# jamornsriwasansak/smallpt-enoki-optix

Hardware: AMD Instinct MI355X
Metric: Mpaths/sec (pixels x spp / s), mitsuba.obj-standin 1024^2 x 64spp, depth 8 (higher is better)
Workload: dtype f32

## Files before the change

include/spt.h:

```cpp
#ifndef SPT_H
#define SPT_H

#include <stddef.h>
#include <stdint.h>

#ifdef __cplusplus
extern "C" {
#endif

typedef int32_t spt_status;
enum {
    SPT_OK = 0,
    SPT_ERR_INVALID = 1,
    SPT_ERR_HIP = 2,
    SPT_ERR_NO_DEVICE = 3,
    SPT_ERR_OOM = 4,
    SPT_ERR_IO = 5,
    SPT_ERR_LIMIT = 6
};

typedef struct spt_scene_t* spt_scene;

typedef struct spt_rays {
    const float* ox; const float* oy; const float* oz;
// ... 22 lines not shown
    float fov_y;
    float film_size_y;
} spt_camera;

enum {
    SPT_RNG_Y_FIRST = 0,
    SPT_RNG_X_FIRST = 1
};

enum {
    SPT_FLAG_TIMING = 1u,
    SPT_FLAG_TRAVERSAL_STATS = 2u,
    SPT_FLAG_FUSED = 4u,
    SPT_FLAG_WAVEFRONT = 8u,
    SPT_FLAG_TIMING_ALL = 16u,
    SPT_FLAG_NO_BOUNCE_CULL = 32u
};

typedef struct spt_render_params {
    uint32_t width, height;
    uint32_t spp;
    uint32_t max_depth;
    spt_camera camera;
    uint32_t tile_index, tile_count, rows_per_group;
    uint32_t wavefront_paths;
    uint32_t rr_start_depth;
    uint32_t rng_order;
    uint64_t rng_initstate;
    float env[3];
    uint32_t flags;
} spt_render_params;
// ... 291 lines not shown

spt_status spt_scene_isect_busy_begin(spt_scene scene);
spt_status spt_scene_isect_busy_end(spt_scene scene, double* busy_ms, uint64_t* launches);
enum { SPT_KERNEL_ISECT = 1u, SPT_KERNEL_DRAIN = 2u };
spt_status spt_scene_kernel_busy(spt_scene scene, uint32_t kernels, double* busy_ms, uint64_t* launches);

uint32_t spt_tile_rows(uint32_t height, uint32_t tile_index, uint32_t tile_count,
                       uint32_t rows_per_group, uint32_t* rows, uint32_t cap);

void spt_default_params(spt_render_params* p);

const char* spt_last_error(void);
const char* spt_version(void);
const char* spt_build_id(void);
void spt_debug_fail_workspace_alloc(int32_t nth);

spt_status spt_obj_load(const char* path, spt_mesh* out);
void spt_mesh_free(spt_mesh* mesh);

typedef struct spt_pbrt_info {
    uint32_t has_camera;
    spt_camera camera;
    float fov_deg;
    uint32_t xres, yres;
    uint32_t has_env;
    float env[3];
    uint64_t shapes;
    uint64_t shapes_skipped;
    uint64_t instances;
} spt_pbrt_info;
// ... 14 lines not shown
```

smallpt-enoki-optix_amd/csrc/kernels.hip:

```cpp
#include <hipcub/hipcub.hpp>
#include <type_traits>

#include "spt_internal.h"

namespace spt {

__device__ __forceinline__ uint32_t wave_uniform(uint32_t v) { return __builtin_amdgcn_readfirstlane(v); }

typedef float spt_f4v __attribute__((ext_vector_type(4)));
typedef float spt_f2v __attribute__((ext_vector_type(2)));
template <bool kNt = false>
__device__ __forceinline__ float4 ldq(const float4* p) {
    if constexpr (kNt) {
        const spt_f4v v = __builtin_nontemporal_load((const spt_f4v*)p);
        return make_float4(v.x, v.y, v.z, v.w);
    } else {
        return *p;
    }
}
template <bool kNt = false>
__device__ __forceinline__ void stq(float4* p, float4 x) {
    if constexpr (kNt) {
        spt_f4v v = {x.x, x.y, x.z, x.w};
        __builtin_nontemporal_store(v, (spt_f4v*)p);
// ... 292 lines not shown
        o = o_;
        const float dx = fabsf(d.x) < kMinDir ? copysignf(kMinDir, d.x) : d.x;
        const float dy = fabsf(d.y) < kMinDir ? copysignf(kMinDir, d.y) : d.y;
        const float dz = fabsf(d.z) < kMinDir ? copysignf(kMinDir, d.z) : d.z;
        ix = __builtin_amdgcn_rcpf(dx); iy = __builtin_amdgcn_rcpf(dy); iz = __builtin_amdgcn_rcpf(dz);
        const uint32_t oct = (ix < 0.0f ? 1u : 0u) | (iy < 0.0f ? 2u : 0u) | (iz < 0.0f ? 4u : 0u);
        const uint32_t oct_inv = oct ^ 7u;
        const uint32_t kz = k >> 4;
        oct_rep = oct_inv * 0x01010101u | ((kz == 2u ? 0u : kz + 1u) << 3);
        tmin = tmin_;
        tbox = box_tmin(tmin_);
        nhits = 1u << (24u + oct_inv);
        ht = tmax_;
    }

    __device__ __forceinline__ bool root_misses(const DeviceScene& sc) {
        nhits = 0;
        tbase = 0;
        thits = 0;
        tbase2 = 0;
        thits2 = 0;
        const uint4* np = sc.nodes8;
        const uint4 w0 = np[0], w1 = np[1], w2 = np[2], w3 = np[3];
        if constexpr (kW == 6) visit_words6(w0, w1, w2, w3);
        else visit_words(w0, w1, w2, w3, np[4]);
        return !(thits | (nhits & 0xff000000u));
    }

    __device__ __forceinline__ void init(const DeviceScene& sc, V3 o_, V3 d, float tmin_, float tmax_, bool anyhit_,
                                         const Lds& L) {
        wr = woop_setup(o_, d);
        spa = (L.wbase + lane_id()) * 4u;
        *wrec(sc, L) = make_uint4(f2u(wr.Sx), f2u(wr.Sy), f2u(wr.Sz), wr.k);
        uint32_t none, zero;
        asm volatile("v_mov_b32 %0, -1" : "=v"(none));
        asm volatile("v_mov_b32 %0, 0" : "=v"(zero));
        *hrec(sc, L) = make_uint4(none, none, zero, zero);
        init_slabs(o_, d, tmin_, tmax_, wr.k);
        anyhit = anyhit_;
        tbase = 0;
        thits = 0;
        tbase2 = 0;
        thits2 = 0;
        done = sc.empty != 0;
    }

    __device__ __forceinline__ uint32_t octx(uint32_t mw) const {
        const uint32_t t8 = mw & (mw >> 1) & 0x08080808u;
        return mw ^ ((t8 - (t8 >> 3)) & oct_rep);
    }

    __device__ __forceinline__ void take_hits(uint32_t hm, uint32_t group, uint32_t tri_base) {
        nhits = (hm & 0xff000000u) | group;
        if (thits) {
            tbase2 = tri_base;
            thits2 = hm & 0x00ffffffu;
// ... 637 lines not shown
        if (!kSpt) {
            const Frame fr = frame_from_normal(sn);
            nd = to_world(fr, cosine_hemisphere(xi_x, xi_y));
        } else {
            float wgt;
            nd = scatter(a.sc, kind, slot, d, no, sn, xi_x, xi_y, wgt);
            tr = tr * wgt; tg = tg * wgt; tb = tb * wgt;
        }
    }
    if constexpr (kCull) {
        __shared__ uint32_t s_wave_cull[kBlock / 64];
        bool gone = false;
        if (emit) {
            CullTr ct;
            ct.init_slabs(no, nd, kRayTmin, kRayTmax, CullTr::kNoRot);
            gone = ct.root_misses(a.sc);
            emit = !gone;
        }
        const uint64_t gball = __ballot(gone);
        if (lane == 0) s_wave_cull[wave] = (uint32_t)__popcll(gball);
        rank = compact_block<kBlock>(a, emit, s_wave_cnt, tid, lane, wave, base);
        if (tid == 0) {
            uint32_t n = 0;
            for (uint32_t w = 0; w < kBlock / 64; w++) n += s_wave_cull[w];
            if (n) atomicAdd(culled + (blockIdx.x % kShards) * kCullStride, (unsigned long long)n);
        }
        if (gone)
            a.sflag[film_slot((meta >> kMetaDepthBits) - a.sample0, pix, a.P, a.chunk_ns, a.work_order)] = 1;
    }
    if (tid == 0) {
        uint32_t off = base;
        for (uint32_t w = 0; w < kBlock / 64; w++) {
            s_wave_off[w] = off;
            off += s_wave_cnt[w];
        }
    }
    __syncthreads();
    if (emit) store_path<kMode, kNt>(a.out, s_wave_off[wave] + rank, no, nd, pix, meta + 1u, tr, tg, tb, lr, lg, lb);
}

template <int kMode, bool kSpt, bool kNt = false>
__global__ __launch_bounds__(kShadeBlock) void shade_kernel(ShadeArgs a) {
    const uint32_t n = *a.count_in;
    if (n < a.drain_below) return;
    const uint32_t nreal = min(gridDim.x, (n + kShadeBlock - 1) / kShadeBlock);
    const uint32_t i =
        (a.xcd_remap && blockIdx.x < nreal ? xcd_block(blockIdx.x, nreal) : blockIdx.x) * kShadeBlock + threadIdx.x;
    shade_block<kMode, kSpt, kNt, kShadeBlock>(a, i < n, QueueSrc<kNt>{a, i});
}

struct CamSrc {
    V3 o, d;
    uint32_t pix, meta;
// ... 100 lines not shown
        dep = dep + t;
        cov = cov + c;
    }
    const float fs = (float)a.spp;
    if (a.albedo_r) a.albedo_r[p] = ar / fs;
    if (a.albedo_g) a.albedo_g[p] = ag / fs;
    if (a.albedo_b) a.albedo_b[p] = ab / fs;
    if (a.normal_x) a.normal_x[p] = nx / fs;
    if (a.normal_y) a.normal_y[p] = ny / fs;
    if (a.normal_z) a.normal_z[p] = nz / fs;
    if (a.depth) a.depth[p] = dep / fs;
    if (a.coverage) a.coverage[p] = cov / fs;
}

template <typename Tr, int kMode, bool kDrain = false, bool kNt = false, bool kList = false, bool kEnv = false,
          bool kNee = false, bool kSky = false, bool kMis = false>
__global__ __launch_bounds__(kIsectBlock)
__attribute__((amdgpu_waves_per_eu(kDrain && kMode == kModeUnit ? (kNt ? SPT_DRAIN_WAVES_NT : SPT_DRAIN_WAVES)
                                   : kDrain ? SPT_DRAIN_WAVES_RGB : SPT_FUSED_WAVES, 8)))
void render_fused_kernel(FusedArgs a) {
    constexpr bool kEmit = kMode == kModeEmit;
    static_assert(!kNee || (kEmit && !kDrain), "light sampling: emitter mode, not the drain");
    static_assert(!kSky || (kNee && kEnv), "sky sampling: the light-sampling lane loop of a scene with a sky image");
    static_assert(!kMis || kNee, "MIS: between the shadow rays and the bounce rays of the light-sampling lane loop");
#if SPT_WAVE_LOG
    const unsigned long long wl_t0 = (unsigned long long)wall_clock64();
#endif
    extern __shared__ uint32_t lds_stack[];
    const Lds L = block_lds(lds_stack);
    uint32_t n = a.count;
    if constexpr (kDrain) {
        if (a.seg_count) {
            n = 0;
            for (uint32_t j = 0; j < kShards; j++) n += a.seg_count[j * kShardStride];
            n = wave_uniform(n);
        } else {
// ... 215 lines not shown
                                        if (traced) {
                                            park[2] = make_float4(dir.x, dir.y, dir.z, sc3.x);
                                            park[3] = make_float4(sc3.y, sc3.z, u2f(lid), 0.0f);
                                            dir = sd;
                                            shadow = true;
                                        }
                                    }
                                }
                            }
                            meta++;
                            if constexpr (kPark) {
                                park[0] = make_float4(thr, thg, thb, lr);
                                park[1] = make_float4(lg, lb, kNee ? u2f(nee_prev) : 0.0f, kMis ? cb : 0.0f);
                            }
                            tr.o = hp;
                            need_init = true;
                            busy = true;
                            cont = true;
                        }
                    }
                }
                if (term) {
                    if (kMode == kModeUnit) {
                        a.sflag[film_slot(sample - a.sample0, pix, a.P, a.pm_ns, a.pm_ns != 0)] = slot == -1 ? 1 : 0;
                    } else {
                        size_t cs;
                        float* f = film_rgb(a.sfilm, sample - a.sample0, pix, a.P, a.pm_ns, a.pm_ns != 0, cs);
                        f[0] = lr;
                        f[cs] = lg;
                        f[2 * cs] = lb;
// ... 28 lines not shown
                        xcd_tries++;
                    }
                    if (xcd_tries >= 8u) { drained = true; break; }
                } else if (pool == pool_end) {
                    uint32_t base = 0;
                    if ((threadIdx.x & 63u) == 0) base = atomicAdd(a.next, a.chunk);
                    base = dyn_base + wave_uniform((uint32_t)__shfl((int)base, 0));
                    if (base >= n) { drained = true; break; }
                    pool = base;
                    pool_end = min(base + a.chunk, n);
                }
                const uint32_t rank = __builtin_amdgcn_mbcnt_hi((uint32_t)(idle >> 32),
                                                                __builtin_amdgcn_mbcnt_lo((uint32_t)idle, 0u));
                const uint32_t take = min((uint32_t)__popcll(idle), pool_end - pool);
                if (kDrain && !busy && !pending && rank < take) {
                    const uint32_t j = a.perm ? a.perm[pool + rank] : pool + rank;
                    const float4 q1 = ldq<kNt>(a.q.q1 + j), q2 = ldq<kNt>(a.q.q2 + j);
                    meta = f2u(q1.w);
                    pix = f2u(q2.w);
                    dir = v3(q2.x, q2.y, q2.z);
                    thr = thg = thb = 1.0f;
                    lr = lg = lb = 0.0f;
                    if (kMode >= kModeAlbedo) {
                        const float4 q0 = ldq<kNt>(a.q.q0 + j);
                        thr = q0.x; thg = q0.y; thb = q0.z;
                        if (kEmit) lr = q0.w;
                    }
                    if (kEmit) {
                        const float2 l = ldq2<kNt>(a.q.rad + j);
                        lg = l.x; lb = l.y;
                    }
                    if constexpr (kPark) {
// ... 27 lines not shown
                }
                if (!kDrain) starts += take;
                pool += take;
#if SPT_WAVE_LOG
                ph[6] += take;
#endif
                idle = __ballot(!busy && !pending);
            }
            if (need_init) {
                if constexpr (kNee) {
                    float tmn = kRayTmin, tmx = kRayTmax;
                    if (shadow) light_shadow_interval(dir, tmn, tmx);
                    if constexpr (kSky)
                        if (skyray) sky_shadow_interval(dir, tmn, tmx);
                    tr.init(a.sc, tr.o, dir, tmn, tmx, kSky && skyray, L);
                } else {
                    tr.init(a.sc, tr.o, dir, kRayTmin, kRayTmax,
                            (meta & ((1u << kMetaDepthBits) - 1u)) + 1u >= a.max_depth && !kEmit, L);
                }
                if (tr.finished()) {
                    busy = false;
                    pending = true;
                }
            }
#if SPT_WAVE_LOG
            const unsigned long long ph_t3 = __builtin_readcyclecounter();
            ph[1] += ph_t3 - ph_t0;
            ph[7] += ph_t3 - ph_t2;
#endif
        }
// ... 521 lines not shown
        else if (mode == kModeEmit) hipLaunchKernelGGL((shade_kernel<kModeEmit, false, true>), g, b, 0, s, a);
        else if (mode == kModeAlbedo && spt) hipLaunchKernelGGL((shade_kernel<kModeAlbedo, true, true>), g, b, 0, s, a);
        else if (mode == kModeAlbedo) hipLaunchKernelGGL((shade_kernel<kModeAlbedo, false, true>), g, b, 0, s, a);
        else hipLaunchKernelGGL((shade_kernel<kModeUnit, false, true>), g, b, 0, s, a);
        return hipGetLastError();
    }
    if (mode == kModeEmit && spt) hipLaunchKernelGGL((shade_kernel<kModeEmit, true>), g, b, 0, s, a);
    else if (mode == kModeEmit) hipLaunchKernelGGL((shade_kernel<kModeEmit, false>), g, b, 0, s, a);
    else if (mode == kModeAlbedo && spt) hipLaunchKernelGGL((shade_kernel<kModeAlbedo, true>), g, b, 0, s, a);
    else if (mode == kModeAlbedo) hipLaunchKernelGGL((shade_kernel<kModeAlbedo, false>), g, b, 0, s, a);
    else hipLaunchKernelGGL((shade_kernel<kModeUnit, false>), g, b, 0, s, a);
    return hipGetLastError();
}

template <typename Tr, int kMode, bool kDrain = false, bool kNt = false, bool kList = false, bool kEnv = false,
          bool kNee = false, bool kSky = false, bool kMis = false>
static hipError_t launch_fused_t(const FusedArgs& a, hipStream_t s, uint32_t* lanes_out) {
    static thread_local size_t cached_lds = 0;
    static thread_local uint32_t cached = 0;
    static thread_local int cached_dev = -1;
    const size_t park = kMode != kModeUnit ? (size_t)kIsectBlock * (kNee ? 64 : 32) : 0;
    const size_t lds = (size_t)a.sc.stack_depth * Tr::kStackWords * kIsectBlock * sizeof(uint32_t) + Tr::kExtraLds + park;
    int dev = 0;
    (void)hipGetDevice(&dev);
    if (!cached || cached_lds != lds || cached_dev != dev) {
        int per_cu = 0, cus = 0;
        if (hipOccupancyMaxActiveBlocksPerMultiprocessor(&per_cu, render_fused_kernel<Tr, kMode, kDrain, kNt, kList, kEnv, kNee, kSky, kMis>,
                                                         kIsectBlock, lds) != hipSuccess || per_cu <= 0)
            per_cu = 1;
        if (hipDeviceGetAttribute(&cus, hipDeviceAttributeMultiprocessorCount, dev) != hipSuccess || cus <= 0)
            cus = 256;
        cached = (uint32_t)(per_cu * cus);
        cached_lds = lds;
        cached_dev = dev;
    }
    const uint32_t scaled = a.grid_q8 ? max(1u, (uint32_t)(((uint64_t)cached * a.grid_q8) >> 8)) : cached;
    const uint32_t blocks = kDrain ? scaled : min(scaled, blocks_for(a.count > 0 ? a.count : 1, kIsectBlock));
    if (lanes_out) *lanes_out = blocks * kIsectBlock;
    hipLaunchKernelGGL((render_fused_kernel<Tr, kMode, kDrain, kNt, kList, kEnv, kNee, kSky, kMis>), dim3(blocks), dim3(kIsectBlock),
                       lds, s, a);
    return hipGetLastError();
}

template <typename Tr, int kMode, bool kDrain = false, bool kNt = false, bool kList = false>
static hipError_t launch_fused_e(const FusedArgs& a, hipStream_t s, uint32_t* lanes_out) {
    if constexpr (kMode == kModeEmit && !kDrain && !kNt) {
        if (a.sc.sky && a.sc.envmap) {
            if (a.sc.mis) return launch_fused_t<Tr, kMode, kDrain, kNt, kList, true, true, true, true>(a, s, lanes_out);
            return launch_fused_t<Tr, kMode, kDrain, kNt, kList, true, true, true>(a, s, lanes_out);
        }
        if (a.sc.lights) {
            if (a.sc.envmap) {
                if (a.sc.mis) return launch_fused_t<Tr, kMode, kDrain, kNt, kList, true, true, false, true>(a, s, lanes_out);
                return launch_fused_t<Tr, kMode, kDrain, kNt, kList, true, true>(a, s, lanes_out);
// ... 60 lines not shown
    if (e) return e;
    return hipcub::DeviceRadixSort::SortPairs(tmp, *tmp_bytes, keys, keys_out, vals, perm, (int)cap, 0, 30, s);
}

hipError_t launch_drain(const FusedArgs& a, int mode, hipStream_t s) {
    if (a.nt) {
        if (mode == kModeEmit) return launch_drain_m<kModeEmit, true>(a, s);
        if (mode == kModeAlbedo) return launch_drain_m<kModeAlbedo, true>(a, s);
        return launch_drain_m<kModeUnit, true>(a, s);
    }
    if (mode == kModeEmit) return launch_drain_m<kModeEmit, false>(a, s);
    if (mode == kModeAlbedo) return launch_drain_m<kModeAlbedo, false>(a, s);
    return launch_drain_m<kModeUnit, false>(a, s);
}

template <typename Tr>
static hipError_t launch_fused_list(const FusedArgs& a, int mode, hipStream_t s, uint32_t* lanes_out) {
    if (mode == kModeEmit) return launch_fused_e<Tr, kModeEmit, false, false, true>(a, s, lanes_out);
    if (mode == kModeAlbedo) return launch_fused_e<Tr, kModeAlbedo, false, false, true>(a, s, lanes_out);
    return launch_fused_e<Tr, kModeUnit, false, false, true>(a, s, lanes_out);
}

hipError_t launch_fused(const FusedArgs& a, int mode, hipStream_t s, uint32_t* lanes_out) {
    if (a.list) {
        if (a.sc.nodes8 && a.sc.node6) return launch_fused_list<Tracer6F>(a, mode, s, lanes_out);
        if (a.sc.nodes8) return launch_fused_list<Tracer8F>(a, mode, s, lanes_out);
        return launch_fused_list<Tracer>(a, mode, s, lanes_out);
    }
    if (a.sc.nodes8 && a.sc.node6) {
        if (mode == kModeEmit) return launch_fused_e<Tracer6F, kModeEmit>(a, s, lanes_out);
// ... 118 lines not shown
```

smallpt-enoki-optix_amd/csrc/render.cpp:

```cpp
#include <hip/hip_runtime.h>

#include <algorithm>
#include <atomic>
#include <cassert>
#include <cmath>
#include <cstddef>
#include <cstring>
#include <mutex>
#include <vector>

#include "render_plan.h"
#include "scene_state.h"

using namespace spt;

namespace {

PathQueue carve_queue(char* base, size_t stride, uint32_t planes) {
    PathQueue q;
    float4* f4 = (float4*)base;
    q.q1 = f4;
    q.q2 = f4 + stride;
    q.q0 = planes > 2 ? f4 + 2 * stride : nullptr;
    q.rad = planes > 3 ? (float2*)(f4 + 3 * stride) : nullptr;
// ... 208 lines not shown

hipError_t create_sub_stream(hipStream_t* s, bool own_queue) {
    if (own_queue) {
        int dev = 0, cus = 0;
        (void)hipGetDevice(&dev);
        if (hipDeviceGetAttribute(&cus, hipDeviceAttributeMultiprocessorCount, dev) == hipSuccess && cus > 0) {
            std::vector<uint32_t> mask(((uint32_t)cus + 31u) / 32u, 0xffffffffu);
            if (cus % 32) mask.back() = (1u << (cus % 32)) - 1u;
            if (hipExtStreamCreateWithCUMask(s, (uint32_t)mask.size(), mask.data()) == hipSuccess) return hipSuccess;
            (void)hipGetLastError();
        }
    }
    return hipStreamCreateWithFlags(s, hipStreamNonBlocking);
}

std::atomic<int32_t> g_fail_ws_alloc{-1};
hipError_t ws_malloc(void** p, size_t bytes) {
    int32_t n = g_fail_ws_alloc.load();
    while (n >= 0 && !g_fail_ws_alloc.compare_exchange_weak(n, n - 1)) {
    }
    if (n == 0) {
        *p = nullptr;
        return hipErrorOutOfMemory;
    }
    return hipMalloc(p, bytes);
}

spt_status ensure_workspace(WorkSet& ws, int nsub, size_t cap, uint32_t pad, uint32_t planes, size_t film_bytes,
                            size_t acc_floats, bool own_queues, bool drain_sort) {
    bool quiet = !ws.used;
// ... 413 lines not shown
struct SubRun {
    IsectQueueArgs ia;
    ShadeArgs sa;
    RefillArgs ra;
    FusedArgs da;
    PathQueue q[2];
    uint32_t drain_T;
    uint32_t known;
    int cur;
    int pending, pend_cur;
    uint64_t pend_it;
    uint64_t limit;
    bool live;
    uint64_t started, sub_begin, sub_end;
    bool lock0;
};

struct RenderJob {
    spt_scene_t* sc;
    const spt_render_params& p;
    const RenderPlan& pl;
    WorkSet& ws;
    RenderSlot& slot;
    float* film_dev;
    const spt_accum* accum;
    uint64_t P;
    uint64_t A;
    const spt_pixel_list* list;
    uint32_t s_begin, s_end;
    const PcgJump *jumps, *cjumps;
// ... 188 lines not shown
    r.ra.work_end = we;
    r.sa.sample0 = s0; r.sa.chunk_ns = ns;
    r.da.sample0 = s0; r.da.pm_ns = pl.pixel_major ? ns : 0;
    r.da.seg_count = nullptr;
    r.da.xcd_next = pl.lane_xcd ? &b.cnt->xcd_next[0][0] : nullptr;
    r.ra.q = r.q[0]; r.ra.surv = &b.cnt->surv[0]; r.ra.cursor_in = nullptr; r.ra.cursor_init = wb;
    r.ra.cursor_out = &b.cnt->cursor[0]; r.ra.qn_out = &b.cnt->qn[0];
    r.ra.surv_clear = nullptr;
    r.ra.casts_in = nullptr;
    r.ra.iter_tag = 1;
    const uint32_t first = (uint32_t)std::min<uint64_t>(b.cap, we - wb);
    r.sub_begin = wb;
    r.sub_end = we;
    r.started = wb + first;
    r.lock0 = j.cfg().lockstep_first && pl.fit && pl.drain_on && !pl.trav_stats && first >= r.drain_T;
    r.ra.book_only = r.lock0 && pl.cam_cast ? 1u : 0u;
    spt_status st;
    if ((st = j.mark(0, sk, [&] { return launch_refill(r.ra, r.ra.book_only ? 1u : first, sk); }))) return st;
    r.ra.book_only = 0;
    r.known = (uint32_t)std::min<uint64_t>(b.cap, r.started - r.sub_begin);
    r.cur = 0;
    r.pending = -1;
    r.pend_cur = 0;
    r.pend_it = 0;
    r.limit = r.started >= r.sub_end ? j.p.max_depth : UINT64_MAX;
    r.live = r.known > 0;
    return SPT_OK;
}

spt_status run_iteration(RenderJob& j, SubRun& r, int k, uint64_t it) {
// ... 15 lines not shown
    r.ia.drain_below = force ? 0xffffffffu : dph ? r.drain_T : 0u;
    r.sa.drain_below = r.ia.drain_below;
    if (force) {
        r.da.q = r.q[c];
        r.da.qcount = &b.cnt->qn[c];
        r.da.drain_below = 0xffffffffu;
        r.da.perm = nullptr;
        if (pl.drain_sort) {
            const size_t cap = b.cap;
            uint32_t* kb = b.sort_buf;
            HIP_TRY(launch_drain_sort(j.sc->dev(), r.q[c], &b.cnt->qn[c], (uint32_t)b.cap, kb, kb + cap, kb + 2 * cap,
                                      kb + 3 * cap, b.sort_tmp, &b.sort_tmp_bytes, sk));
            r.da.perm = kb + 3 * cap;
        }
        r.da.count_queue = 1;
        if ((st = j.mark(4, sk, [&] { return launch_drain(r.da, mode, sk); }))) return st;
        r.da.count_queue = 0;
        j.drain_launches++;
        r.cur = nx;
        r.live = false;
        return SPT_OK;
    }
    const bool lockstep = it == 0 && r.lock0;
    if (lockstep) j.slot.rs.lockstep_casts += r.known;
    bool sharded = false;
    if (lockstep && pl.cam_cast) {
        sharded = pl.cam_shards && !pl.drain_sort && j.forced_at(r, it + 1);
        CameraCastArgs ca;
        ca.r = r.ra;
        ca.s = r.sa;
        ca.s.in = r.q[c];
        ca.s.out = r.q[nx];
        ca.s.hits = nullptr;
        ca.s.count_in = &b.cnt->qn[c];
        ca.s.count_out = sharded ? &b.cnt->surv_shard[0][0] : &b.cnt->surv[nx];
        ca.s.shard_items = sharded ? r.known : 0u;
        ca.n = r.known;
        unsigned long long* const culled = pl.bounce_cull && !ca.s.sc.empty ? &j.slot.dev->culled[0][0] : nullptr;
        if ((st = j.mark(1, sk, [&] { return launch_camera_cast(ca, mode, sk, culled); }))) return st;
        if (sharded) {
            r.da.seg_count = &b.cnt->surv_shard[0][0];
            r.da.seg_items = r.known;
            r.da.seg_block = kIsectBlock;
            r.da.xcd_next = &b.cnt->xcd_next[0][0];
        }
    } else if ((st = j.mark(1, sk, [&] {
                   if (lockstep) return launch_isect_lockstep(r.ia, r.known, sk);
                   return pl.trav_stats ? launch_isect_queue_stats(r.ia, r.known, sk)
                                        : launch_isect_queue(r.ia, r.known, sk);
               })))
        return st;
    r.sa.in = r.q[c]; r.sa.out = r.q[nx];
    r.sa.count_in = &b.cnt->qn[c];
// ... 227 lines not shown
    rs.streams = (uint32_t)K;
    rs.fused = pl.fused ? 1u : 0u;
    rs.drain_refill_idle = !pl.fused && pl.drain_on ? pl.drain_idle : 0u;
    slot->regen_base = std::min<uint64_t>(C, job.A * p.spp);
    slot->ticket = sc->ws.next_ticket++;
    slot->pending = true;
    *ticket_out = slot->ticket;
    return SPT_OK;
}

}

extern "C" {

void spt_debug_fail_workspace_alloc(int32_t nth) { g_fail_ws_alloc.store(nth < 0 ? -1 : nth); }

spt_status spt_render_async(spt_scene sc, const spt_render_params* pp, float* film_dev, void* caller,
                            uint64_t* ticket_out) {
    return render_enqueue(sc, pp, film_dev, nullptr, false, caller, ticket_out);
}

spt_status spt_render_accum_async(spt_scene sc, const spt_render_params* pp, const spt_accum* acc, void* caller,
                                  uint64_t* ticket_out) {
    return render_enqueue(sc, pp, nullptr, acc, true, caller, ticket_out);
}

spt_status spt_render_accum(spt_scene sc, const spt_render_params* pp, const spt_accum* acc,
                            spt_render_stats* stats_out, void* stream) {
    uint64_t ticket = 0;
    spt_status st = spt_render_accum_async(sc, pp, acc, stream, &ticket);
// ... 120 lines not shown
```

smallpt-enoki-optix_amd/csrc/render_plan.h:

```cpp
#pragma once
#include <stdint.h>

#include <algorithm>

#include "../../include/spt.h"

namespace spt {

constexpr int kMaxStreams = 4;
constexpr uint64_t kHitBytes = 16;
constexpr uint64_t kMinRetryPaths = 1u << 16;
constexpr uint64_t kPixelMajorMinSceneBytes = 256ull << 20;
constexpr uint64_t kPixelMajorMinFusedPaths = 16ull << 20;
constexpr uint64_t kPixelMajorMinWaveSceneBytes = 4ull << 20;
constexpr uint64_t kPixelMajorMaxWaveTilePx = 4ull << 20;
constexpr uint32_t kDefaultWavefrontPaths = 1u << 25;
constexpr uint64_t kPixelMajorWavefrontPaths = 24ull << 20;
constexpr uint32_t kDefaultDrainQ8 = 1024;
constexpr uint64_t kDefaultFusedMaxPaths = 1ull << 20;
constexpr uint64_t kDefaultFitPaths = 1ull << 28;
constexpr uint32_t kDefaultDrainCasts = 1;
constexpr uint32_t kDrainIdleSpheres = 56;
constexpr uint32_t kDrainIdleStream = 40;
constexpr uint32_t kDrainIdleCached = 24;
// ... 26 lines not shown
    uint64_t C = 0;
    int K = 1;
    uint64_t Ck = 0;
    uint32_t chunk = 1;
    uint32_t pixel_major = 0, queue_nt = 0, drain_idle = 0;
    int mode = 0;
    bool own_queues = false;
    bool trav_stats = false;
    bool drain_on = false;
    bool drain_sort = false;
    bool sort_buffers = false;
    bool cam_cast = false;
    bool cam_shards = false;
    bool lane_xcd = false;
    bool bounce_cull = false;
};

inline RenderPlan plan_render(const RenderPlanIn& in, uint64_t fit_limit) {
    const spt_config& cfg = *in.cfg;
    const uint64_t P = in.P, A = in.A ? in.A : in.P, jobs = A * in.spp;
    RenderPlan pl;
    pl.mode = in.mode;
    bool& fused = pl.fused;
    uint64_t &C = pl.C, &fit_paths = pl.fit_paths, &mem_paths = pl.mem_paths;
    uint32_t& fit_chunk = pl.fit_chunk;
    C = in.wavefront_paths ? in.wavefront_paths : cfg.wavefront_paths;

    const bool trav_stats = pl.trav_stats = (in.flags & SPT_FLAG_TRAVERSAL_STATS) != 0;
    const uint64_t fused_max = in.wavefront_paths ? in.wavefront_paths : cfg.fused_max_paths;
    fused = cfg.pipeline == SPT_PIPELINE_AUTO ? jobs <= fused_max : cfg.pipeline == SPT_PIPELINE_FUSED;
// ... 44 lines not shown
    if ((uint64_t)K > C) K = (int)C;
    pl.Ck = (C + K - 1) / K;
    const uint64_t budget = cfg.film_budget_bytes;
    uint32_t& chunk = pl.chunk = (uint32_t)std::max<uint64_t>(
        1, std::min<uint64_t>(std::min<uint64_t>(in.spp, budget / (in.film_unit * P)), 0x7fffffffull / P));
    if (fit_chunk) chunk = std::min(chunk, fit_chunk);
    if (mem_paths != UINT64_MAX) chunk = (uint32_t)std::max<uint64_t>(1, std::min<uint64_t>(chunk, mem_paths / P));
    pl.drain_on = cfg.drain_q8 != 0 && !trav_stats;
    pl.lane_xcd = (cfg.xcd_remap & 4u) != 0;
    pl.drain_sort = pl.drain_on && cfg.drain_sort != 0 && in.wide_nodes;
    pl.sort_buffers = !fused && cfg.drain_q8 != 0 && cfg.drain_sort != 0 && in.wide_nodes;
    pl.cam_cast = cfg.lockstep_first >= 2 && in.wide_nodes;
    pl.cam_shards = pl.cam_cast && cfg.lockstep_first >= 3;
    pl.bounce_cull = pl.cam_shards && !(in.flags & SPT_FLAG_NO_BOUNCE_CULL) && in.mode == 0 && in.nsph == 0 &&
                     scene_bytes < kPixelMajorMinSceneBytes;
    return pl;
}

}
```

smallpt-enoki-optix_amd/csrc/spt_internal.h:

```cpp
#pragma once
#include <hip/hip_runtime.h>
#include <stdint.h>

#include <vector>

#include "spt_math.h"
#include "shard_base.h"

namespace spt {

constexpr uint32_t kMaxDepthCasts = 64;
constexpr uint32_t kNode8Quads = 8;
constexpr uint32_t kTriQuads = 4;
constexpr uint32_t kTriFloats = 16;
constexpr uint32_t kTriIdFloat = 15;
SPT_HD void tri_record_fill(float* rec, const float* v9, uint32_t id) {
    for (int k = 0; k < 3; k++) {
        rec[5 * k] = v9[3 * k];
        rec[5 * k + 1] = v9[3 * k + 1];
        rec[5 * k + 2] = v9[3 * k + 2];
        rec[5 * k + 3] = v9[3 * k];
        rec[5 * k + 4] = v9[3 * k + 1];
    }
    rec[kTriIdFloat] = u2f(id);
// ... 513 lines not shown
    const uint32_t rb = H - band * B < B ? H - band * B : B;
    const uint32_t cb = off / (B * rb);
    const uint32_t inner = off - cb * B * rb;
    const uint32_t cw = W - cb * B < B ? W - cb * B : B;
    const uint32_t r = inner / cw;
    lx = cb * B + (inner - r * cw);
    ly = band * B + r;
}

hipError_t launch_isect_queue(const IsectQueueArgs& a, uint32_t grid_items, hipStream_t s);
hipError_t launch_isect_lockstep(const IsectQueueArgs& a, uint32_t grid_items, hipStream_t s);
hipError_t launch_isect_queue_stats(const IsectQueueArgs& a, uint32_t grid_items, hipStream_t s);
hipError_t launch_isect_public(const IsectPublicArgs& a, hipStream_t s);
hipError_t launch_fused(const FusedArgs& a, int mode, hipStream_t s, uint32_t* lanes_out);
hipError_t launch_drain(const FusedArgs& a, int mode, hipStream_t s);
hipError_t launch_drain_sort(const DeviceScene& sc, const PathQueue& q, const uint32_t* count, uint32_t cap,
                             uint32_t* keys, uint32_t* vals, uint32_t* keys_out, uint32_t* perm, void* tmp,
                             size_t* tmp_bytes, hipStream_t s);
uint32_t isect_queue_lanes(const IsectQueueArgs& a);
hipError_t launch_shade(const ShadeArgs& a, int mode, uint32_t grid_items, hipStream_t s);
hipError_t launch_camera_cast(const CameraCastArgs& a, int mode, hipStream_t s, unsigned long long* culled = nullptr);
hipError_t launch_refill(const RefillArgs& a, uint32_t grid_items, hipStream_t s);
hipError_t launch_aov(const AovArgs& a, hipStream_t s);
hipError_t launch_denoise(const DenoiseArgs& a, hipStream_t s);
hipError_t launch_denoise_var_init(const float* var3, float* v0, uint32_t P, hipStream_t s);
hipError_t launch_denoise_var(const DenoiseVarArgs& a, hipStream_t s);
hipError_t launch_resolve(const float* sfilm, float* acc, float* out, uint32_t P, uint32_t nsamples,
                          uint32_t first_chunk, uint32_t last_chunk, uint32_t spp, uint32_t order,
                          unsigned long long* unwritten, hipStream_t s);
hipError_t launch_resolve_flags(const uint8_t* sflag, float* acc, float* out, uint32_t P, uint32_t nsamples,
// ... 86 lines not shown
```

smallpt-enoki-optix_amd/sptamd/_lib.py:

```python
from __future__ import annotations

import ctypes
import os
from ctypes import POINTER, c_char_p, c_double, c_float, c_int32, c_uint8, c_uint32, c_uint64, c_void_p

PKG_ROOT = os.path.dirname(os.path.dirname(os.path.abspath(__file__)))
REPO_ROOT = os.path.dirname(PKG_ROOT)
LIB_PATH = os.environ.get("SPT_LIB") or os.path.join(PKG_ROOT, "build", "libspt.so")

SPT_OK = 0
SPT_ERR_INVALID, SPT_ERR_HIP, SPT_ERR_NO_DEVICE, SPT_ERR_OOM, SPT_ERR_IO, SPT_ERR_LIMIT = 1, 2, 3, 4, 5, 6
SPT_RNG_Y_FIRST = 0
SPT_RNG_X_FIRST = 1
SPT_FLAG_TIMING = 1
SPT_FLAG_TRAVERSAL_STATS = 2
SPT_FLAG_FUSED = 4
SPT_FLAG_WAVEFRONT = 8
SPT_FLAG_TIMING_ALL = 16
SPT_FLAG_NO_BOUNCE_CULL = 32
PCG32_DEFAULT_STATE = 0x853C49E6748FEA9B
SPT_BUILD_AUTO, SPT_BUILD_HOST_SAH, SPT_BUILD_GPU_PLOC = 0, 1, 2

EXPORTED = [
    "spt_init", "spt_scene_create", "spt_scene_create_ex", "spt_scene_set_albedo", "spt_scene_set_emission", "spt_scene_get_stats",
    "spt_scene_destroy", "spt_intersect", "spt_hit_info_compute", "spt_render", "spt_render_async", "spt_render_wait",
    "spt_tile_rows", "spt_default_params", "spt_last_error", "spt_version", "spt_build_id",
    "spt_obj_load", "spt_mesh_free", "spt_pfm_write", "spt_pbrt_load",
    "spt_default_config", "spt_scene_create_cfg", "spt_scene_set_config", "spt_scene_get_config",
    "spt_bvh_build_stats", "spt_scene_set_texture", "spt_scene_set_spheres", "spt_scene_set_material_kinds",
    "spt_scene_save", "spt_scene_load", "spt_scene_cache_info",
    "spt_scene_isect_busy_begin", "spt_scene_isect_busy_end", "spt_scene_kernel_busy",
    "spt_debug_fail_workspace_alloc",
    "spt_render_aov", "spt_default_denoise_params", "spt_denoise_scratch_bytes", "spt_denoise",
    "spt_scene_update_geometry", "spt_scene_update_geometry_device", "spt_scene_get_refit_stats",
    "spt_render_accum", "spt_render_accum_async",
    "spt_default_denoise_var_params", "spt_denoise_var_scratch_bytes", "spt_denoise_var",
    "spt_default_adapt_params", "spt_adapt_select_scratch_bytes", "spt_adapt_select", "spt_render_accum_list",
    "spt_scene_set_envmap", "spt_envmap_from_latlong", "spt_pfm_read", "spt_pfm_free",
    "spt_scene_set_light_sampling", "spt_scene_get_light_sampling", "spt_light_table_build",
    "spt_scene_get_shadow_casts",
    "spt_scene_set_sky_sampling", "spt_scene_get_sky_sampling", "spt_sky_table_build",
    "spt_scene_set_mis", "spt_scene_get_mis",
]
SPT_MAT_DIFFUSE, SPT_MAT_MIRROR, SPT_MAT_GLASS = 0, 1, 2
SPT_PIPELINE_AUTO, SPT_PIPELINE_WAVEFRONT, SPT_PIPELINE_FUSED = 0, 1, 2
SPT_WORK_AUTO, SPT_WORK_SAMPLE_MAJOR, SPT_WORK_PIXEL_MAJOR = 0, 1, 2
SPT_QUEUE_CACHE_AUTO, SPT_QUEUE_CACHE_CACHED, SPT_QUEUE_CACHE_STREAM = 0, 1, 2
# ... 161 lines not shown
        "spt_scene_destroy": (i32, [vp]),
        "spt_intersect": (i32, [vp, POINTER(Rays), vp, u32, POINTER(Hits), u32, i32, vp]),
        "spt_hit_info_compute": (i32, [vp, POINTER(Rays), POINTER(Hits), vp, u32, u32, POINTER(HitInfo), vp]),
        "spt_render": (i32, [vp, POINTER(RenderParams), vp, POINTER(RenderStats), vp]),
        "spt_render_async": (i32, [vp, POINTER(RenderParams), vp, vp, POINTER(u64)]),
        "spt_render_wait": (i32, [vp, u64, POINTER(RenderStats)]),
        "spt_scene_isect_busy_begin": (i32, [vp]),
        "spt_scene_isect_busy_end": (i32, [vp, POINTER(ctypes.c_double), POINTER(u64)]),
        "spt_scene_kernel_busy": (i32, [vp, u32, POINTER(ctypes.c_double), POINTER(u64)]),
        "spt_tile_rows": (u32, [u32, u32, u32, u32, vp, u32]),
        "spt_default_params": (None, [POINTER(RenderParams)]),
        "spt_last_error": (c_char_p, []),
        "spt_version": (c_char_p, []),
        "spt_build_id": (c_char_p, []),
        "spt_debug_fail_workspace_alloc": (None, [ctypes.c_int32]),
        "spt_obj_load": (i32, [c_char_p, POINTER(Mesh)]),
        "spt_mesh_free": (None, [POINTER(Mesh)]),
        "spt_pbrt_load": (i32, [c_char_p, POINTER(Mesh), POINTER(PbrtInfo)]),
        "spt_pfm_write": (i32, [c_char_p, vp, vp, vp, u32, u32]),
        "spt_default_config": (None, [POINTER(Config)]),
        "spt_scene_create_cfg": (i32, [vp, vp, u64, u64, vp, vp, u64, vp, vp, u64, vp, POINTER(Config), POINTER(vp)]),
        "spt_scene_set_config": (i32, [vp, POINTER(Config)]),
        "spt_scene_get_config": (i32, [vp, POINTER(Config)]),
        "spt_bvh_build_stats": (i32, [vp, u64, POINTER(Config), POINTER(SceneStats)]),
        "spt_scene_set_texture": (i32, [vp, u32, vp, u32, u32]),
        "spt_scene_set_spheres": (i32, [vp, vp, vp, u32]),
        "spt_scene_set_material_kinds": (i32, [vp, vp, u32]),
        "spt_scene_save": (i32, [vp, c_char_p, vp, u64]),
        "spt_scene_load": (i32, [c_char_p, POINTER(vp), vp, u64, POINTER(u64)]),
        "spt_scene_cache_info": (i32, [c_char_p, POINTER(SceneStats), POINTER(Config), POINTER(u64)]),
# ... 167 lines not shown
```

Before: 7037.

## Hand off root-node visit results from bounce cull to the drain kernel

The bounce-cull step in the camera-cast kernel already tests each emitted ray against the BVH root. That root-hit word is now stored per queued path and handed to a new drain kernel variant, which seeds the traversal state from it instead of re-visiting the root. This removes one root-node fetch and box test per ray. In exchange it adds a per-path 4-byte store and load, another kernel instantiation, and a rule that the queue is read without the sort permutation when the hand-off is active.

```diff
diff --git a/include/spt.h b/include/spt.h
--- a/include/spt.h
+++ b/include/spt.h
@@ -60,7 +60,8 @@
     SPT_FLAG_FUSED = 4u,
     SPT_FLAG_WAVEFRONT = 8u,
     SPT_FLAG_TIMING_ALL = 16u,
-    SPT_FLAG_NO_BOUNCE_CULL = 32u
+    SPT_FLAG_NO_BOUNCE_CULL = 32u,
+    SPT_FLAG_NO_ROOT_HANDOFF = 64u
 };
 
 typedef struct spt_render_params {
@@ -382,6 +383,7 @@
 const char* spt_version(void);
 const char* spt_build_id(void);
 void spt_debug_fail_workspace_alloc(int32_t nth);
+uint64_t spt_debug_root_drain_launches(void);
 
 spt_status spt_obj_load(const char* path, spt_mesh* out);
 void spt_mesh_free(spt_mesh* mesh);
diff --git a/smallpt-enoki-optix_amd/csrc/kernels.hip b/smallpt-enoki-optix_amd/csrc/kernels.hip
--- a/smallpt-enoki-optix_amd/csrc/kernels.hip
+++ b/smallpt-enoki-optix_amd/csrc/kernels.hip
@@ -330,7 +330,9 @@
         ht = tmax_;
     }
 
-    __device__ __forceinline__ bool root_misses(const DeviceScene& sc) {
+    __device__ __forceinline__ bool root_misses(const DeviceScene& sc) { return !root_visit(sc); }
+
+    __device__ __forceinline__ uint32_t root_visit(const DeviceScene& sc) {
         nhits = 0;
         tbase = 0;
         thits = 0;
@@ -340,9 +342,18 @@
         const uint4 w0 = np[0], w1 = np[1], w2 = np[2], w3 = np[3];
         if constexpr (kW == 6) visit_words6(w0, w1, w2, w3);
         else visit_words(w0, w1, w2, w3, np[4]);
-        return !(thits | (nhits & 0xff000000u));
-    }
-
+        return thits | (nhits & 0xff000000u);
+    }
+
+    __device__ __forceinline__ void enter_root(const DeviceScene& sc, uint32_t word) {
+        const uint32_t* n0 = (const uint32_t*)sc.nodes8;
+        const uint32_t group = kW == 6 ? n0[6] & 0x00ffffffu : n0[4];
+        tbase = kW == 6 ? n0[3] : n0[5];
+        nhits = (word & 0xff000000u) | group;
+        thits = word & 0x00ffffffu;
+    }
+
+    template <bool kRoot = false>
     __device__ __forceinline__ void init(const DeviceScene& sc, V3 o_, V3 d, float tmin_, float tmax_, bool anyhit_,
                                          const Lds& L) {
         wr = woop_setup(o_, d);
@@ -355,7 +366,11 @@
         init_slabs(o_, d, tmin_, tmax_, wr.k);
         anyhit = anyhit_;
         tbase = 0;
-        thits = 0;
+        if constexpr (kRoot) {
+            if (thits) enter_root(sc, thits);
+        } else {
+            thits = 0;
+        }
         tbase2 = 0;
         thits2 = 0;
         done = sc.empty != 0;
@@ -1023,7 +1038,8 @@
         if (emit) {
             CullTr ct;
             ct.init_slabs(no, nd, kRayTmin, kRayTmax, CullTr::kNoRot);
-            gone = ct.root_misses(a.sc);
+            slot = (int32_t)ct.root_visit(a.sc);
+            gone = !slot;
             emit = !gone;
         }
         const uint64_t gball = __ballot(gone);
@@ -1046,6 +1062,8 @@
     }
     __syncthreads();
     if (emit) store_path<kMode, kNt>(a.out, s_wave_off[wave] + rank, no, nd, pix, meta + 1u, tr, tg, tb, lr, lg, lb);
+    if constexpr (kCull)
+        if (emit && a.hits) ((uint32_t*)a.hits)[s_wave_off[wave] + rank] = (uint32_t)slot;
 }
 
 template <int kMode, bool kSpt, bool kNt = false>
@@ -1176,12 +1194,13 @@
 }
 
 template <typename Tr, int kMode, bool kDrain = false, bool kNt = false, bool kList = false, bool kEnv = false,
-          bool kNee = false, bool kSky = false, bool kMis = false>
+          bool kNee = false, bool kSky = false, bool kMis = false, bool kRoot = false>
 __global__ __launch_bounds__(kIsectBlock)
 __attribute__((amdgpu_waves_per_eu(kDrain && kMode == kModeUnit ? (kNt ? SPT_DRAIN_WAVES_NT : SPT_DRAIN_WAVES)
                                    : kDrain ? SPT_DRAIN_WAVES_RGB : SPT_FUSED_WAVES, 8)))
 void render_fused_kernel(FusedArgs a) {
     constexpr bool kEmit = kMode == kModeEmit;
+    static_assert(!kRoot || (kDrain && kMode == kModeUnit && !kNt), "the root hand-off: the unit-mode cached-queue drain");
     static_assert(!kNee || (kEmit && !kDrain), "light sampling: emitter mode, not the drain");
     static_assert(!kSky || (kNee && kEnv), "sky sampling: the light-sampling lane loop of a scene with a sky image");
     static_assert(!kMis || kNee, "MIS: between the shadow rays and the bounce rays of the light-sampling lane loop");
@@ -1427,6 +1446,7 @@
                                 park[1] = make_float4(lg, lb, kNee ? u2f(nee_prev) : 0.0f, kMis ? cb : 0.0f);
                             }
                             tr.o = hp;
+                            if constexpr (kRoot) tr.thits = 0;
                             need_init = true;
                             busy = true;
                             cont = true;
@@ -1485,8 +1505,9 @@
                                                                 __builtin_amdgcn_mbcnt_lo((uint32_t)idle, 0u));
                 const uint32_t take = min((uint32_t)__popcll(idle), pool_end - pool);
                 if (kDrain && !busy && !pending && rank < take) {
-                    const uint32_t j = a.perm ? a.perm[pool + rank] : pool + rank;
+                    const uint32_t j = kRoot ? pool + rank : a.perm ? a.perm[pool + rank] : pool + rank;
                     const float4 q1 = ldq<kNt>(a.q.q1 + j), q2 = ldq<kNt>(a.q.q2 + j);
+                    if constexpr (kRoot) tr.thits = a.perm[j];
                     meta = f2u(q1.w);
                     pix = f2u(q2.w);
                     dir = v3(q2.x, q2.y, q2.z);
@@ -1544,6 +1565,9 @@
                     if constexpr (kSky)
                         if (skyray) sky_shadow_interval(dir, tmn, tmx);
                     tr.init(a.sc, tr.o, dir, tmn, tmx, kSky && skyray, L);
+                } else if constexpr (kRoot) {
+                    tr.template init<true>(a.sc, tr.o, dir, kRayTmin, kRayTmax,
+                                           (meta & ((1u << kMetaDepthBits) - 1u)) + 1u >= a.max_depth, L);
                 } else {
                     tr.init(a.sc, tr.o, dir, kRayTmin, kRayTmax,
                             (meta & ((1u << kMetaDepthBits) - 1u)) + 1u >= a.max_depth && !kEmit, L);
@@ -2095,7 +2119,7 @@
 }
 
 template <typename Tr, int kMode, bool kDrain = false, bool kNt = false, bool kList = false, bool kEnv = false,
-          bool kNee = false, bool kSky = false, bool kMis = false>
+          bool kNee = false, bool kSky = false, bool kMis = false, bool kRoot = false>
 static hipError_t launch_fused_t(const FusedArgs& a, hipStream_t s, uint32_t* lanes_out) {
     static thread_local size_t cached_lds = 0;
     static thread_local uint32_t cached = 0;
@@ -2106,7 +2130,7 @@
     (void)hipGetDevice(&dev);
     if (!cached || cached_lds != lds || cached_dev != dev) {
         int per_cu = 0, cus = 0;
-        if (hipOccupancyMaxActiveBlocksPerMultiprocessor(&per_cu, render_fused_kernel<Tr, kMode, kDrain, kNt, kList, kEnv, kNee, kSky, kMis>,
+        if (hipOccupancyMaxActiveBlocksPerMultiprocessor(&per_cu, render_fused_kernel<Tr, kMode, kDrain, kNt, kList, kEnv, kNee, kSky, kMis, kRoot>,
                                                          kIsectBlock, lds) != hipSuccess || per_cu <= 0)
             per_cu = 1;
         if (hipDeviceGetAttribute(&cus, hipDeviceAttributeMultiprocessorCount, dev) != hipSuccess || cus <= 0)
@@ -2118,7 +2142,7 @@
     const uint32_t scaled = a.grid_q8 ? max(1u, (uint32_t)(((uint64_t)cached * a.grid_q8) >> 8)) : cached;
     const uint32_t blocks = kDrain ? scaled : min(scaled, blocks_for(a.count > 0 ? a.count : 1, kIsectBlock));
     if (lanes_out) *lanes_out = blocks * kIsectBlock;
-    hipLaunchKernelGGL((render_fused_kernel<Tr, kMode, kDrain, kNt, kList, kEnv, kNee, kSky, kMis>), dim3(blocks), dim3(kIsectBlock),
+    hipLaunchKernelGGL((render_fused_kernel<Tr, kMode, kDrain, kNt, kList, kEnv, kNee, kSky, kMis, kRoot>), dim3(blocks), dim3(kIsectBlock),
                        lds, s, a);
     return hipGetLastError();
 }
@@ -2209,6 +2233,13 @@
     return launch_drain_m<kModeUnit, false>(a, s);
 }
 
+hipError_t launch_drain_root(const FusedArgs& a, hipStream_t s) {
+    if (!a.sc.nodes8 || a.sc.empty || a.nt || !a.perm || !a.seg_count) return hipErrorInvalidValue;
+    if (a.sc.node6)
+        return launch_fused_t<Tracer6F, kModeUnit, true, false, false, false, false, false, false, true>(a, s, nullptr);
+    return launch_fused_t<Tracer8F, kModeUnit, true, false, false, false, false, false, false, true>(a, s, nullptr);
+}
+
 template <typename Tr>
 static hipError_t launch_fused_list(const FusedArgs& a, int mode, hipStream_t s, uint32_t* lanes_out) {
     if (mode == kModeEmit) return launch_fused_e<Tr, kModeEmit, false, false, true>(a, s, lanes_out);
diff --git a/smallpt-enoki-optix_amd/csrc/render.cpp b/smallpt-enoki-optix_amd/csrc/render.cpp
--- a/smallpt-enoki-optix_amd/csrc/render.cpp
+++ b/smallpt-enoki-optix_amd/csrc/render.cpp
@@ -246,6 +246,7 @@
     return hipStreamCreateWithFlags(s, hipStreamNonBlocking);
 }
 
+std::atomic<uint64_t> g_root_drain_launches{0};
 std::atomic<int32_t> g_fail_ws_alloc{-1};
 hipError_t ws_malloc(void** p, size_t bytes) {
     int32_t n = g_fail_ws_alloc.load();
@@ -689,6 +690,7 @@
     bool live;
     uint64_t started, sub_begin, sub_end;
     bool lock0;
+    bool root_words;
 };
 
 struct RenderJob {
@@ -907,6 +909,7 @@
     r.sub_end = we;
     r.started = wb + first;
     r.lock0 = j.cfg().lockstep_first && pl.fit && pl.drain_on && !pl.trav_stats && first >= r.drain_T;
+    r.root_words = false;
     r.ra.book_only = r.lock0 && pl.cam_cast ? 1u : 0u;
     spt_status st;
     if ((st = j.mark(0, sk, [&] { return launch_refill(r.ra, r.ra.book_only ? 1u : first, sk); }))) return st;
@@ -952,7 +955,13 @@
             r.da.perm = kb + 3 * cap;
         }
         r.da.count_queue = 1;
-        if ((st = j.mark(4, sk, [&] { return launch_drain(r.da, mode, sk); }))) return st;
+        const bool root = r.root_words;
+        r.root_words = false;
+        if (root) r.da.perm = (const uint32_t*)b.hits;
+        if ((st = j.mark(4, sk, [&] { return root ? launch_drain_root(r.da, sk) : launch_drain(r.da, mode, sk); })))
+            return st;
+        if (root) g_root_drain_launches.fetch_add(1);
+        r.da.perm = nullptr;
         r.da.count_queue = 0;
         j.drain_launches++;
         r.cur = nx;
@@ -975,6 +984,11 @@
         ca.s.shard_items = sharded ? r.known : 0u;
         ca.n = r.known;
         unsigned long long* const culled = pl.bounce_cull && !ca.s.sc.empty ? &j.slot.dev->culled[0][0] : nullptr;
+        r.root_words = sharded && culled && pl.root_handoff && !r.da.nt;
+        if (r.root_words) {
+            assert((uint64_t)shard_base(kShards, r.known, kIsectBlock) * sizeof(uint32_t) <= kHitBytes * (uint64_t)b.cap);
+            ca.s.hits = (const float4*)b.hits;
+        }
         if ((st = j.mark(1, sk, [&] { return launch_camera_cast(ca, mode, sk, culled); }))) return st;
         if (sharded) {
             r.da.seg_count = &b.cnt->surv_shard[0][0];
@@ -1232,6 +1246,7 @@
 extern "C" {
 
 void spt_debug_fail_workspace_alloc(int32_t nth) { g_fail_ws_alloc.store(nth < 0 ? -1 : nth); }
+uint64_t spt_debug_root_drain_launches(void) { return g_root_drain_launches.load(); }
 
 spt_status spt_render_async(spt_scene sc, const spt_render_params* pp, float* film_dev, void* caller,
                             uint64_t* ticket_out) {
diff --git a/smallpt-enoki-optix_amd/csrc/render_plan.h b/smallpt-enoki-optix_amd/csrc/render_plan.h
--- a/smallpt-enoki-optix_amd/csrc/render_plan.h
+++ b/smallpt-enoki-optix_amd/csrc/render_plan.h
@@ -64,6 +64,7 @@
     bool cam_shards = false;
     bool lane_xcd = false;
     bool bounce_cull = false;
+    bool root_handoff = false;
 };
 
 inline RenderPlan plan_render(const RenderPlanIn& in, uint64_t fit_limit) {
@@ -138,6 +139,7 @@
     pl.cam_shards = pl.cam_cast && cfg.lockstep_first >= 3;
     pl.bounce_cull = pl.cam_shards && !(in.flags & SPT_FLAG_NO_BOUNCE_CULL) && in.mode == 0 && in.nsph == 0 &&
                      scene_bytes < kPixelMajorMinSceneBytes;
+    pl.root_handoff = pl.bounce_cull && !(in.flags & SPT_FLAG_NO_ROOT_HANDOFF);
     return pl;
 }
 
diff --git a/smallpt-enoki-optix_amd/csrc/spt_internal.h b/smallpt-enoki-optix_amd/csrc/spt_internal.h
--- a/smallpt-enoki-optix_amd/csrc/spt_internal.h
+++ b/smallpt-enoki-optix_amd/csrc/spt_internal.h
@@ -551,6 +551,7 @@
 hipError_t launch_isect_public(const IsectPublicArgs& a, hipStream_t s);
 hipError_t launch_fused(const FusedArgs& a, int mode, hipStream_t s, uint32_t* lanes_out);
 hipError_t launch_drain(const FusedArgs& a, int mode, hipStream_t s);
+hipError_t launch_drain_root(const FusedArgs& a, hipStream_t s);
 hipError_t launch_drain_sort(const DeviceScene& sc, const PathQueue& q, const uint32_t* count, uint32_t cap,
                              uint32_t* keys, uint32_t* vals, uint32_t* keys_out, uint32_t* perm, void* tmp,
                              size_t* tmp_bytes, hipStream_t s);
diff --git a/smallpt-enoki-optix_amd/sptamd/_lib.py b/smallpt-enoki-optix_amd/sptamd/_lib.py
--- a/smallpt-enoki-optix_amd/sptamd/_lib.py
+++ b/smallpt-enoki-optix_amd/sptamd/_lib.py
@@ -18,6 +18,7 @@
 SPT_FLAG_WAVEFRONT = 8
 SPT_FLAG_TIMING_ALL = 16
 SPT_FLAG_NO_BOUNCE_CULL = 32
+SPT_FLAG_NO_ROOT_HANDOFF = 64
 PCG32_DEFAULT_STATE = 0x853C49E6748FEA9B
 SPT_BUILD_AUTO, SPT_BUILD_HOST_SAH, SPT_BUILD_GPU_PLOC = 0, 1, 2
 
@@ -30,7 +31,7 @@
     "spt_bvh_build_stats", "spt_scene_set_texture", "spt_scene_set_spheres", "spt_scene_set_material_kinds",
     "spt_scene_save", "spt_scene_load", "spt_scene_cache_info",
     "spt_scene_isect_busy_begin", "spt_scene_isect_busy_end", "spt_scene_kernel_busy",
-    "spt_debug_fail_workspace_alloc",
+    "spt_debug_fail_workspace_alloc", "spt_debug_root_drain_launches",
     "spt_render_aov", "spt_default_denoise_params", "spt_denoise_scratch_bytes", "spt_denoise",
     "spt_scene_update_geometry", "spt_scene_update_geometry_device", "spt_scene_get_refit_stats",
     "spt_render_accum", "spt_render_accum_async",
@@ -222,6 +223,7 @@
         "spt_version": (c_char_p, []),
         "spt_build_id": (c_char_p, []),
         "spt_debug_fail_workspace_alloc": (None, [ctypes.c_int32]),
+        "spt_debug_root_drain_launches": (ctypes.c_uint64, []),
         "spt_obj_load": (i32, [c_char_p, POINTER(Mesh)]),
         "spt_mesh_free": (None, [POINTER(Mesh)]),
         "spt_pbrt_load": (i32, [c_char_p, POINTER(Mesh), POINTER(PbrtInfo)]),
```

After: 7146 (median of 6 runs). 1.02x the previous value.
